# atx/padne

Measured on AMD Instinct MI355X. Metric: CG solves/s, higher is better.
Workload: dtype f64; 1 GPU; C4 8-layer N=10M: 8-layer jittered triangular Laplacian, 9999392 nodes, via-ring stitched, 1 A source/sink, amg-PCG to rtol 1e-12; n_unknowns=9999391, nnz_per_rank=69955225, rows_per_rank=9999391, parallelism=layer-partitioned x1

## Files before the change

### padne_amd/_hip.py

```python
from __future__ import annotations

import ctypes as C
import weakref
import os
import sys
from dataclasses import dataclass

import numpy as np

_HERE = os.path.dirname(os.path.abspath(__file__))
LIB_PATH = os.path.join(_HERE, "libpadne_hip.so")

OK = 0
E_INVALID, E_HIP, E_NOMEM, E_NONMANIFOLD, E_NOTCONVERGED, E_COMM, E_BREAKDOWN, E_TOOLARGE, E_NOCOARSEN = \
    -1, -2, -3, -4, -5, -6, -7, -8, -9


class HipUnavailableError(RuntimeError):
    """libpadne_hip.so cannot be loaded or no MI355X is visible."""


class HipError(RuntimeError):
    def __init__(self, code: int, message: str):
        super().__init__(f"libpadne_hip error {code}: {message}")
# ... 109 lines not shown
                                       _PF64, _PF64, _PF64]),
    "padne_sampler_stats": (C.c_int, [_P, C.c_int32, _PI64, _PF64]),
    "padne_spmv_algorithmic_bytes": (_I64, [_P]),
    "padne_spmv_time": (C.c_int, [_P, _P, _P, _P, C.c_int, C.c_int, _PF64]),
}

TEST_SIGNATURES = {
    "padne_team_create": (C.c_int, [C.c_int, C.POINTER(_P)]),
    "padne_team_destroy": (C.c_int, [_P]),
    "padne_team_abort": (C.c_int, [_P]),
    "padne_ctx_join_team": (C.c_int, [_P, _P, C.c_int]),
    "padne_csr_split_tiles": (C.c_int, [_P, C.c_int, _PI64, _PI64]),
    "padne_ctx_lockstep_groups": (C.c_int, [_P, _PI64]),
    "padne_asm_second_path_count": (C.c_int, [_PI64]),
    "padne_ctx_halo_exchange_time": (C.c_int, [_P, C.c_int32, C.POINTER(C.c_double)]),
    "padne_ctx_reload_options": (C.c_int, [_P]),
}

PROBE_SIGNATURES = {
    "padne_test_product": (C.c_int, [_P, _P, C.c_int32, _I64, C.c_int32, C.c_int32, C.c_int32, C.c_int32, _P, _P, _P, _P, _P,
                                     _P, _P, _P, _P, C.c_double, _P, _PF64, _I64, _PI32]),
}

_lib = None


def load_library(path: str | None = None) -> C.CDLL:
    global _lib
    if _lib is not None and path is None:
        return _lib
    p = path or LIB_PATH
    if not os.path.exists(p):
        raise HipUnavailableError(
            f"{p} not found: build it with `python -m padne_amd.build` (hipcc --offload-arch=gfx950). "
            "padne_amd has no CPU fallback.")
    if "torch" in sys.modules:
        pass
    try:
        lib = C.CDLL(p, mode=C.RTLD_GLOBAL)
    except OSError as exc:
        raise HipUnavailableError(f"cannot load {p}: {exc}") from exc
    for name, (res, args) in list(SIGNATURES.items()) + list(TEST_SIGNATURES.items()) + list(PROBE_SIGNATURES.items()):
        fn = getattr(lib, name)
        fn.restype = res
        fn.argtypes = args
    if lib.padne_abi_version() != 1:
        raise HipUnavailableError("libpadne_hip.so ABI version mismatch; rebuild it")
    if path is None:
        _lib = lib
    return lib


def _check(rc: int) -> None:
    if rc == OK:
        return
    msg = (load_library().padne_last_error() or b"").decode("utf-8", "replace")
    if rc == E_NONMANIFOLD:
        raise ValueError(msg or "Non-manifold mesh")
    if rc == E_INVALID:
        raise ValueError(msg)
    if rc == E_NOMEM:
        raise MemoryError(msg)
    if rc == E_TOOLARGE:
        raise OverflowError(msg)
    if rc == E_NOTCONVERGED:
# ... 811 lines not shown
        _check(self.ctx._lib.padne_csr_shape(h, C.byref(nr), C.byref(nc), C.byref(nnz)))
        indptr = np.empty(nr.value + 1, dtype=np.int32)
        indices = np.empty(nnz.value, dtype=np.int32)
        data = np.empty(nnz.value, dtype=np.float64)
        _check(self.ctx._lib.padne_csr_to_host(self.ctx._h, h, _ptr(indptr, _PI32), _ptr(indices, _PI32), _ptr(data, _PF64)))
        return sp.csr_matrix((data, indices, indptr), shape=(nr.value, nc.value))

    def amg_shapes(self):
        out = []
        for level in range(32):
            entry = {}
            for which, code in (("A", 0), ("P", 1), ("R", 2)):
                h = _P()
                if self.ctx._lib.padne_amg_level(self.ctx._h, self._h, level, code, C.byref(h)) != OK:
                    continue
                nr, nc, nnz = C.c_int64(), C.c_int64(), C.c_int64()
                _check(self.ctx._lib.padne_csr_shape(h, C.byref(nr), C.byref(nc), C.byref(nnz)))
                entry[which] = (nr.value, nc.value, nnz.value)
            if "A" not in entry:
                break
            out.append(entry)
        return out

    def split_tiles(self, level: int = -1):
        a, b = C.c_int64(), C.c_int64()
        _check(self.ctx._lib.padne_csr_split_tiles(self._h, int(level), C.byref(a), C.byref(b)))
        return a.value, b.value

    def amg_apply(self, r) -> np.ndarray:
        r = _f64(r)
        if r.shape[0] != self.shape[0]:
            raise ValueError("dimension mismatch")
        z = np.empty_like(r)
        _check(self.ctx._lib.padne_amg_apply(self.ctx._h, self._h, _ptr(r, _PF64), _ptr(z, _PF64)))
        return z

    @staticmethod
    def _opts(rtol, atol, max_iter, check_every, guess, time_spmv=False, precond="jacobi", rebuild=False) -> SolveOpts:
        pc = {"jacobi": 0, "amg": 1, 0: 0, 1: 1}[precond]
        return SolveOpts(float(rtol), float(atol), int(max_iter), pc, int(check_every),
                         (1 if guess else 0) | (2 if time_spmv else 0) | (4 if rebuild else 0))

    def solve_spd(self, b, *, rtol=1e-12, atol=0.0, max_iter=200000, check_every=0, x0=None,
                  raise_on_fail=True, precond="amg", rebuild=False) -> SolveResult:
        b = _f64(b)
        n = self.shape[0] if self.ctx.halo_n_owned is None else self.ctx.halo_n_owned
# ... 27 lines not shown
```

### padne_amd/build.py

```python
from __future__ import annotations

import os
import shutil
import subprocess
import sys

HERE = os.path.dirname(os.path.abspath(__file__))
CSRC = os.path.join(HERE, "csrc")
LIB = os.path.join(HERE, "libpadne_hip.so")
SOURCES = ["capi.hip", "spmv.hip", "spmm.hip", "pcg.hip", "assemble.hip", "comm.hip", "amg.hip", "generate.hip", "kkt.hip", "sample.hip", "error.hip", "refine.hip"]
HEADERS = ["common.hpp", "face.hpp", os.path.join("..", "..", "include", "padne_hip.h"),
           os.path.join("..", "..", "include", "padne_hip_test.h"), os.path.join("..", "..", "include", "padne_hip_probe.h")]
ARCH = "gfx950"
FLAGS = ["-O3", "-std=c++17", "-fPIC", f"--offload-arch={ARCH}", "-ffp-contract=off",
         "-fno-fast-math", "-Wall", "-Wno-unused-function", "-Wno-unused-value", "-Wno-unused-result"]


def hipcc() -> str:
    exe = shutil.which("hipcc") or "/opt/rocm/bin/hipcc"
    if not os.path.exists(exe):
        raise RuntimeError("hipcc not found: libpadne_hip.so cannot be built")
    return exe


def needs_build() -> bool:
    if not os.path.exists(LIB):
        return True
    t = os.path.getmtime(LIB)
    deps = [os.path.join(CSRC, s) for s in SOURCES + HEADERS] + [os.path.abspath(__file__)]
    return any(os.path.getmtime(d) > t for d in deps)


def build(force: bool = False, verbose: bool = True) -> str:
    if not force and not needs_build():
        return LIB
# ... 26 lines not shown
```

### padne_amd/csrc/amg.hip

```cpp
#include "common.hpp"

#include <functional>
#include <type_traits>
#include <memory>

#include <algorithm>
#include <chrono>
#include <math.h>
#include <stdlib.h>
#include <string.h>

namespace padne {

struct AmgLevel {
    const padne_csr *A = nullptr;
    padne_csr *A_owned = nullptr;
    padne_csr *P = nullptr;
    padne_csr *R = nullptr;
    padne_csr *W = nullptr;
    double lambda = 2.0;
    double jac = 0.0;
    long long n = 0;
    double *b = nullptr, *xa = nullptr, *xb = nullptr, *tmp = nullptr;
    float *b8 = nullptr, *xa8 = nullptr, *xb8 = nullptr, *tmp8 = nullptr;
    HaloPlan halo;
    int32_t *export_owned = nullptr;
    std::vector<int> export_host;
    padne_csr *P_halo = nullptr;
    float *e_ext = nullptr;
};

struct Amg {
    padne_ctx *ctx = nullptr;
    std::vector<AmgLevel> levels;
    double *coarse_inv = nullptr;
    int n_coarse = 0;
    bool f32 = false;
    float *coarse_inv32 = nullptr;
    bool dist = false;
    padne_csr *tail = nullptr;
    int n_pad = 0;
    long long tail_n = 0, tail_off = 0;
    int *seg_off = nullptr;
    double *coarse_gather = nullptr;
// ... 58 lines not shown
__device__ __forceinline__ unsigned int prio32_of(int i) {
    unsigned int h = (unsigned int)i & 0x7fffffffu;
    h = (h * 0x5bd1e995u) & 0x7fffffffu;
    h ^= h >> 15;
    h = (h * 0x2c1b3c6du) & 0x7fffffffu;
    h ^= h >> 13;
    h = (h * 0x297a2d39u) & 0x7fffffffu;
    h ^= h >> 16;
    return h + 1u;
}

__device__ __forceinline__ bool strong(double a, double di, double dj, double theta2) {
    return a * a * di * dj >= theta2;
}

__device__ __forceinline__ int xw_position(const int4 d, const int run, const int c) {
    int pos = 0;
    if (c >= d.z && c < d.z + run) pos = 2 * run + (c - d.z);
    if (c >= d.y && c < d.y + run) pos = run + (c - d.y);
    if (c >= d.x && c < d.x + run) pos = c - d.x;
    return pos;
}

__global__ __launch_bounds__(256) void strength_mark(int n, int n_wtiles, const int *__restrict__ rowptr,
                                                     const int *__restrict__ cols, const double *__restrict__ vals,
                                                     const double *__restrict__ dinv, double theta2,
                                                     int *__restrict__ scol, double *__restrict__ bound_partial,
                                                     const int4 *__restrict__ xw_desc = nullptr,
                                                     const unsigned char *__restrict__ xw_lidx = nullptr,
                                                     const int xw_run = 0, unsigned char *__restrict__ spos = nullptr,
                                                     float *__restrict__ vals32 = nullptr) {
    constexpr int CH = 512;
    __shared__ unsigned char rid_all[4 * CH];
    __shared__ double pv_all[4 * CH];
    __shared__ double red[4], red2[4];
    const int lane = threadIdx.x & 63, w = threadIdx.x >> 6;
    unsigned char *rid = rid_all + w * CH;
    double *pv = pv_all + w * CH;
    const XcdSweep sw = xcd_sweep(n_wtiles, 4, w);
    double my_max = 0.0, my_plain = 0.0;
    for (long long wt = sw.t0; wt < sw.t1; wt += sw.stride) {
        const int row0 = (int)wt * 64;
        const int row1 = min(row0 + 64, n);
        const int r = row0 + lane;
        int rs = 0, re = 0;
        double di = 0.0;
        if (r < row1) {
            rs = rowptr[r];
            re = rowptr[r + 1];
            di = dinv[r];
        }
        const int k0 = __shfl(rs, 0, 64);
        const int k1 = __shfl(re, row1 - row0 - 1, 64);
        double dF = r < row1 ? 1.0 / di : 1.0, off_strong = 0.0, off_all = 0.0, abs_all = 0.0;
        int4 dsc = make_int4(0, 0, 0, 0);
        if (spos != nullptr) dsc = xw_desc[wt];
        const bool windowed = spos != nullptr && dsc.w != 0;
        const int self_pos = windowed ? xw_position(dsc, xw_run, r) : 0;
        for (int base = k0; base < k1; base += CH) {
            const int lo = max(rs, base), hi = min(re, base + CH);
            for (int k = lo; k < hi; ++k) rid[k - base] = (unsigned char)lane;
            asm volatile("s_waitcnt lgkmcnt(0)" ::: "memory");
            __builtin_amdgcn_wave_barrier();
#pragma unroll
            for (int q = 0; q < CH / 64; ++q) {
                const int e = base + lane + 64 * q;
                const int rl = e < k1 ? rid[e - base] : 0;
                const double dr = __shfl(di, rl, 64);
                const int sp = __shfl(self_pos, rl, 64);
                if (e < k1) {
                    const int i = row0 + rl;
                    const int c = cols[e];
                    const double v = vals[e];
                    if (vals32 != nullptr) vals32[e] = (float)v;
                    const bool st = c != i && strong(v, dr, dinv[c], theta2);
                    scol[e] = st ? c : i;
                    if (windowed) spos[e] = st ? xw_lidx[e] : (unsigned char)sp;
                    if (bound_partial != nullptr) {
                        rid[e - base] = (unsigned char)(rl | (c == i ? 0x40 : 0) | (st ? 0x80 : 0));
                        pv[e - base] = v;
// ... 420 lines not shown
            for (int u = 0; u < 8; ++u) aj[u] = (k0 + u < k1 && j[u] != i) ? agg_in[j[u]] : -1;
#pragma unroll
            for (int u = 0; u < 8; ++u) {
                const double w = fabs(v[u]);
                if (aj[u] >= 0 && w > best) {
                    best = w;
                    a = aj[u];
                }
            }
        }
        for (int k = k0 + 8; k < k1; ++k) {
            const int j = scol[k];
            if (j == i) continue;
            const int aj = agg_in[j];
            if (aj < 0) continue;
            const double w = fabs(vals[k]);
            if (w > best) {
                best = w;
                a = aj;
            }
        }
    }
    agg_out[i] = a;
}

__global__ void flag_unaggregated(int n, const int *__restrict__ agg, int *__restrict__ flag) {
    const int i = blockIdx.x * blockDim.x + threadIdx.x;
    if (i < n) flag[i] = agg[i] < 0 ? 1 : 0;
}

__global__ void agg_singletons(int n, const int *__restrict__ scan, const long long *__restrict__ base_dev, int *__restrict__ agg) {
    const int i = blockIdx.x * blockDim.x + threadIdx.x;
    if (i < n && agg[i] < 0) agg[i] = (int)*base_dev + scan[i];
}

__global__ __launch_bounds__(256) void gershgorin_kernel(int n, const int *__restrict__ rowptr,
                                                         const double *__restrict__ vals,
                                                         const double *__restrict__ dinv,
                                                         double *__restrict__ partial_max) {
    __shared__ double red[256];
    double m = 0.0;
    for (int i = blockIdx.x * 256 + threadIdx.x; i < n; i += gridDim.x * 256) {
        double s = 0.0;
        for (int k = rowptr[i]; k < rowptr[i + 1]; ++k) s += fabs(vals[k]);
        s *= fabs(dinv[i]);
        m = s > m ? s : m;
// ... 1419 lines not shown
        out2[0] = red[0][0];
        out2[1] = red[1][0];
    }
}

static int gershgorin(padne_ctx *ctx, const padne_csr *A, double *lambda, bool filtered = false) {
    const int g = (int)std::min<long long>((A->n_rows + 255) / 256, 1024);
    double *part = ctx->partials + 6 * kMaxPartials;
    if (filtered)
        hipLaunchKernelGGL(gershgorin_filtered_kernel, dim3(g > 0 ? g : 1), dim3(256), 0, ctx->stream, (int)A->n_rows,
                           A->rowptr, A->cols, A->vals, A->dinv, kTheta * kTheta, part);
    else
        hipLaunchKernelGGL(gershgorin_kernel, dim3(g > 0 ? g : 1), dim3(256), 0, ctx->stream, (int)A->n_rows, A->rowptr,
                           A->vals, A->dinv, part);
    hipLaunchKernelGGL(fold_max2_kernel, dim3(1), dim3(256), 0, ctx->stream, (const double *)part, (const double *)nullptr,
                       g > 0 ? g : 1, part + kMaxPartials - 2);
    PADNE_HIP_CHECK(hipGetLastError());
    double h[2] = {0.0, 0.0};
    PADNE_TRY(read_back(ctx, part + kMaxPartials - 2, sizeof(h), h));
    double m = h[0];
    if (!(m > 0.0) || !(m < 1e6)) m = 2.0;
    *lambda = m;
    return PADNE_OK;
}

static int aggregate(padne_ctx *ctx, Scratch &sc, const padne_csr *A, int **agg_out, int *n_agg, double *lambda_f = nullptr,
                     double *lambda_plain = nullptr, unsigned char **spos_out = nullptr, int **scol_out = nullptr,
                     float *vals32_out = nullptr) {
    hipStream_t s = ctx->stream;
    const int n = (int)A->n_rows;
    const double theta2 = kTheta * kTheta;
    signed char *state = nullptr;
    unsigned int *w0 = nullptr, *w1 = nullptr, *w2 = nullptr;
    int *flag = nullptr, *scan = nullptr, *agg0 = nullptr, *agg1 = nullptr, *counter = nullptr;
    PADNE_TRY(sc.alloc(&state, (size_t)n));
    PADNE_TRY(sc.alloc(&w0, (size_t)n));
    PADNE_TRY(sc.alloc(&w1, (size_t)n));
    PADNE_TRY(sc.alloc(&w2, (size_t)n));
    PADNE_TRY(sc.alloc(&flag, (size_t)n + 1));
    PADNE_TRY(sc.alloc(&scan, (size_t)n + 1));
    PADNE_TRY(sc.alloc(&agg0, (size_t)n));
    PADNE_TRY(sc.alloc(&agg1, (size_t)n));
    constexpr int kMaxRounds = 256;
    PADNE_TRY(sc.alloc(&counter, (size_t)2 * kMaxRounds + 4));
    const dim3 g(nblk(n)), b(256);
    const int *srow = A->rowptr;
    int *scol = nullptr;
    PADNE_TRY(sc.alloc(&scol, (size_t)(A->nnz > 0 ? A->nnz : 1)));
    const int n_wt = (n + 63) / 64;
    int gm_x = std::min(2048, (n_wt + 3) / 4 > 0 ? (n_wt + 3) / 4 : 1);
    if (gm_x >= kNumXcd) gm_x -= gm_x % kNumXcd;
    const dim3 gm((unsigned)gm_x);
    double *bound_part = lambda_f != nullptr ? ctx->partials + 6 * kMaxPartials : nullptr;
    double *bound2 = nullptr;
    if (lambda_f != nullptr) PADNE_TRY(sc.alloc(&bound2, 2));
    const bool xw = A->xw_state == 1 && A->xw_run <= 85;
    unsigned char *spos = nullptr;
    if (xw) {
        PADNE_TRY(sc.alloc(&spos, (size_t)A->nnz + kPadNnz));
    }
    static_assert(kPadNnz >= 2 * kMaxRounds + 4, "one grid for everything the start clears");
    hipLaunchKernelGGL(mis_init_words, dim3(nblk(std::max(n, kPadNnz))), b, 0, s, n, w0, state, counter, 2 * kMaxRounds + 4,
                       spos != nullptr ? spos + A->nnz : (unsigned char *)nullptr, kPadNnz);
    hipLaunchKernelGGL(strength_mark, gm, b, 0, s, n, n_wt, A->rowptr, A->cols, A->vals, A->dinv, theta2, scol, bound_part,
                       xw ? A->xw_desc : (const int4 *)nullptr, xw ? (const unsigned char *)A->xw_lidx : (const unsigned char *)nullptr,
                       xw ? A->xw_run : 0, spos, vals32_out);
    PADNE_HIP_CHECK(hipGetLastError());
    const bool long_rows = !xw && n <= 65536 && A->nnz >= 24LL * n;
    auto launch_round = [&](int *open_counter) {
        if (xw) {
            hipLaunchKernelGGL((nbr_max_xw<unsigned int, false>), gm, b, 0, s, n, n_wt, srow, scol, spos, A->xw_desc, A->xw_run,
                               (const unsigned int *)w0, w1, (unsigned int *)nullptr, (signed char *)nullptr, (int *)nullptr);
            hipLaunchKernelGGL((nbr_max_xw<unsigned int, true>), gm, b, 0, s, n, n_wt, srow, scol, spos, A->xw_desc, A->xw_run,
                               (const unsigned int *)w1, (unsigned int *)nullptr, w0, state, open_counter);
        } else if (long_rows) {
            hipLaunchKernelGGL(nbr_max_wpr<unsigned int>, dim3((unsigned)((n + 3) / 4)), b, 0, s, n, srow, (const int *)scol,
                               (const unsigned int *)w0, w1);
            hipLaunchKernelGGL(nbr_max_wpr<unsigned int>, dim3((unsigned)((n + 3) / 4)), b, 0, s, n, srow, (const int *)scol,
                               (const unsigned int *)w1, w2);
            hipLaunchKernelGGL(mis_decide, dim3(std::min<unsigned>(g.x, 1024u)), b, 0, s, n, w0, w2, state, open_counter);
        } else {
            hipLaunchKernelGGL(nbr_max<unsigned int>, gm, b, 0, s, n, n_wt, srow, scol, w0, w1);
            hipLaunchKernelGGL(nbr_max<unsigned int>, gm, b, 0, s, n, n_wt, srow, scol, w1, w2);
            hipLaunchKernelGGL(mis_decide, dim3(std::min<unsigned>(g.x, 1024u)), b, 0, s, n, w0, w2, state, open_counter);
        }
    };
    if (lambda_f != nullptr)
        hipLaunchKernelGGL(fold_max2_kernel, dim3(1), dim3(256), 0, s, (const double *)bound_part,
                           (const double *)(bound_part + kMaxPartials), (int)gm.x, bound2);
    double h_bound2[2] = {0.0, 0.0};
    bool bound_pending = lambda_f != nullptr;
    auto count_back = [&](const int *dev_count, int *host_count) -> int {
        if (!bound_pending) return read_back(ctx, dev_count, sizeof(int), host_count);
        bound_pending = false;
        return read_back2(ctx, dev_count, sizeof(int), host_count, bound2, sizeof(h_bound2), h_bound2);
    };
    int open_count = n;
    int round = 0;
    const bool compact_ok = A->nnz <= 16LL * n;
    const int full_batch = n > 200000 ? 1 : 4;
    while (round < kMaxRounds && open_count > 0 && (!compact_ok || round < 2 || open_count > n / 8)) {
        const int reps = (round == 0 && compact_ok && full_batch < 2) ? 2 : full_batch;
        for (int rep = 0; rep < reps && round < kMaxRounds; ++rep, ++round) {
            launch_round(counter + round);
        }
        PADNE_HIP_CHECK(hipGetLastError());
        PADNE_TRY(count_back(counter + round - 1, &open_count));
    }
    if (open_count > 0) {
        int *list_a = (int *)w1, *list_b = (int *)w2;
        unsigned int *m2 = nullptr;
        PADNE_TRY(sc.alloc(&m2, (size_t)open_count));
// ... 18 lines not shown
                hipLaunchKernelGGL(mis_decide_list, gl, b, 0, s, counters + cur, list_a, m2, w0, state, list_b, counters + cur + 1);
                std::swap(list_a, list_b);
                ++cur;
            }
            PADNE_HIP_CHECK(hipGetLastError());
            PADNE_TRY(count_back(counters + cur, &cnt));
        }
        open_count = cnt;
    }
    PADNE_REQUIRE(open_count == 0, "independent-set rounds did not terminate");
    if (lambda_f != nullptr) {
        if (bound_pending) PADNE_TRY(read_back(ctx, bound2, sizeof(h_bound2), h_bound2));
        double m = h_bound2[0], mp = h_bound2[1];
        if (!(m > 0.0) || !(m < 1e6)) m = 2.0;
        if (!(mp > 0.0) || !(mp < 1e6)) mp = 2.0;
        *lambda_f = m;
        if (lambda_plain != nullptr) *lambda_plain = mp;
    }
    hipLaunchKernelGGL(flag_state, g, b, 0, s, n, state, flag, 1);
    ScanTicket t_roots, t_single;
    long long h_roots[2] = {0, 0}, h_single[2] = {0, 0};
    PADNE_TRY(scan_i32_begin(ctx, flag, scan, n, &t_roots, true));
    hipLaunchKernelGGL(agg_from_roots, g, b, 0, s, n, state, scan, agg0);
    hipLaunchKernelGGL(agg_join, g, b, 0, s, n, srow, scol, A->vals, agg0, agg1);
    hipLaunchKernelGGL(agg_join, g, b, 0, s, n, srow, scol, A->vals, agg1, agg0);
    hipLaunchKernelGGL(flag_unaggregated, g, b, 0, s, n, agg0, flag);
    int rc_scan = scan_i32_begin(ctx, flag, scan, n, &t_single, true);
    if (rc_scan == PADNE_OK && t_roots.bs != nullptr)
        hipLaunchKernelGGL(agg_singletons, g, b, 0, s, n, scan, (const long long *)(t_roots.bs + t_roots.nb), agg0);
    const int rc_roots = scan_i32_end(ctx, &t_roots, h_roots);
    if (rc_scan == PADNE_OK) rc_scan = scan_i32_end(ctx, &t_single, h_single);
    PADNE_TRY(rc_roots);
    PADNE_TRY(rc_scan);
    PADNE_HIP_CHECK(hipGetLastError());
    const long long n_roots = h_roots[0], n_single = h_single[0];
    PADNE_REQUIRE(n_roots >= 0 && n_single >= 0 && n_roots + n_single < 2147483647LL, "aggregate count out of range");
    *agg_out = agg0;
    *n_agg = (int)(n_roots + n_single);
    if (spos_out != nullptr) *spos_out = spos;
    if (scol_out != nullptr) *scol_out = scol;
    return PADNE_OK;
}

template <int CAP>
__global__ __launch_bounds__(128) void prolong_rows_lds(int n, const int *__restrict__ rowptr, const int *__restrict__ cols,
                                                        const double *__restrict__ vals, const double *__restrict__ dinv,
                                                        double theta2, double omega, const int *__restrict__ agg,
                                                        const int *__restrict__ slot_ptr, long long *__restrict__ key,
// ... 565 lines not shown
        keep_slots->valid = true;
        sc.disown(first);
        sc.disown(key);
        sc.disown(val);
        if (C != nullptr) *C = nullptr;
        return PADNE_OK;
    }
    auto trampoline = [](void *f) -> int { return (*static_cast<const std::function<int()> *>(f))(); };
    return csr_from_slots(ctx, n, Y->n_cols, row_begin != nullptr ? row_begin : slot_ptr, key, val, row_len, C,
                          while_multiplying != nullptr ? +trampoline : nullptr, const_cast<std::function<int()> *>(while_multiplying));
}

__global__ void slot_row_lengths(int n, const int *__restrict__ begin, const int *__restrict__ end, int *__restrict__ len) {
    const int i = blockIdx.x * blockDim.x + threadIdx.x;
    if (i < n) len[i] = end[i] - begin[i];
}

__global__ __launch_bounds__(256) void w_from_slots_kernel(int n, const int *__restrict__ ap_begin,
                                                           const long long *__restrict__ ap_key,
                                                           const double *__restrict__ ap_val, const int *__restrict__ pr,
                                                           const int *__restrict__ pc, const double *__restrict__ pv,
                                                           const double *__restrict__ dinv, const double c,
                                                           const int *__restrict__ wr, int *__restrict__ wc,
                                                           float *__restrict__ wv) {
    __shared__ int rp_all[4][65];
    __shared__ int sp_all[4][65];
    const int lane = threadIdx.x & 63, w = threadIdx.x >> 6;
    int *rp = rp_all[w], *sp = sp_all[w];
    const long long n_wt = ((long long)n + 63) / 64;
    for (long long wt = (long long)blockIdx.x * 4 + w; wt < n_wt; wt += (long long)gridDim.x * 4) {
        const long long r0 = wt * 64;
        const int nr = (int)((n - r0) < 64 ? (n - r0) : 64);
        if (lane <= nr) rp[lane] = wr[r0 + lane];
        if (lane < nr) sp[lane] = ap_begin[r0 + lane];
        if (lane == 0 && nr == 64) rp[64] = wr[r0 + 64];
        asm volatile("s_waitcnt lgkmcnt(0)" ::: "memory");
        __builtin_amdgcn_wave_barrier();
        const int d0 = rp[0], d1 = rp[nr];
        for (int k = d0 + lane; k < d1; k += 64) {
            int lo = 0, hi = nr;
            while (hi - lo > 1) {
                const int mid = (lo + hi) >> 1;
                if (rp[mid] <= k) lo = mid; else hi = mid;
            }
            const int i = (int)r0 + lo;
            const int src = sp[lo] + (k - rp[lo]);
            const int col = (int)(ap_key[src] >> 32);
            double v = -c * dinv[i] * ap_val[src];
            const I2u be = *reinterpret_cast<const I2u *>(pr + i);
            if (be.y - be.x <= 4) {
                const I4u c4 = *reinterpret_cast<const I4u *>(pc + be.x);
                const D2u p0 = *reinterpret_cast<const D2u *>(pv + be.x), p1 = *reinterpret_cast<const D2u *>(pv + be.x + 2);
                const int ln = be.y - be.x;
                if (ln > 0 && c4.x == col) v = p0.x + v;
                if (ln > 1 && c4.y == col) v = p0.y + v;
// ... 19 lines not shown
                            double c, padne_csr **W_out, int grid_cap = 0, bool with_plan = true) {
    hipStream_t s = ctx->stream;
    const int n = (int)A->n_rows;
    Scratch sc(ctx);
    int *len = nullptr;
    PADNE_TRY(sc.alloc(&len, (size_t)n + 1));
    struct CsrDrop { void operator()(padne_csr *m) const { if (m) padne_csr_destroy(m); } };
    std::unique_ptr<padne_csr, CsrDrop> w_owner(new padne_csr());
    padne_csr *W = w_owner.get();
    W->n_rows = n;
    W->n_cols = P->n_cols;
    W->nnz = n_slots;
    W->device = ctx->device;
    W->owner = ctx;
    W->hierarchy_operator = true;
    W->xw_state = -1;
    W->rowptr = (int32_t *)pool_alloc(ctx, sizeof(int32_t) * ((size_t)n + 1));
    W->cols = (int32_t *)pool_alloc(ctx, sizeof(int32_t) * ((size_t)n_slots + kPadNnz));
    W->vals32 = (float *)pool_alloc(ctx, sizeof(float) * ((size_t)n_slots + kPadNnz));
    if (!W->rowptr || !W->cols || !W->vals32) return PADNE_E_NOMEM;
    hipLaunchKernelGGL(slot_row_lengths, dim3(nblk(n)), dim3(256), 0, s, n, ap.begin, ap.end, len);
    PADNE_HIP_CHECK(hipGetLastError());
    PADNE_TRY(exclusive_scan_i32_async(ctx, len, W->rowptr, n));
    unsigned gw = nblk(((long long)n + 63) / 64, 4);
    if (grid_cap > 0 && gw > (unsigned)grid_cap) gw = (unsigned)grid_cap;
    hipLaunchKernelGGL(w_from_slots_kernel, dim3(gw), dim3(256), 0, s, n, ap.begin, ap.key, ap.val,
                       P->rowptr, P->cols, P->vals, A->dinv, c, (const int *)W->rowptr, W->cols, W->vals32);
    PADNE_HIP_CHECK(hipGetLastError());
    W->xw_state = 0;
    if (with_plan) PADNE_TRY(csr_build_xw_plan_wide(ctx, W, grid_cap));
    if (W->xw_state != 1) W->xw_state = -1;
    *W_out = w_owner.release();
    return PADNE_OK;
}

static int dense_inverse(padne_ctx *ctx, const padne_csr *A, double **inv_out) {
    hipStream_t s = ctx->stream;
    const int n = (int)A->n_rows;
    Scratch sc(ctx);
    double *W = nullptr, *W2 = nullptr, *inv = nullptr;
    PADNE_TRY(sc.alloc(&W, (size_t)n * n));
    PADNE_TRY(sc.alloc(&W2, (size_t)n * n));
    inv = (double *)pool_alloc(ctx, sizeof(double) * (size_t)(n > 0 ? n : 1) * (size_t)(n > 0 ? n : 1));
    if (inv == nullptr) return PADNE_E_NOMEM;
    if (n > 0) {
        hipLaunchKernelGGL(dense_from_csr, dim3(n), dim3(256), 0, s, n, A->rowptr, A->cols, A->vals, W);
        const dim3 ge(nblk(n), (unsigned)((n + kGjStrip - 1) / kGjStrip));
        double *src = W, *dst = W2;
        const bool mfma = !ctx->opt.gj_vector && n > kGjM;
        if (mfma) {
// ... 210 lines not shown
            if (want_f32) PADNE_TRY(csr_build_f32(aux, const_cast<padne_csr *>(A)));
            if (want_f32 && L.P != nullptr && !w_expected) PADNE_TRY(csr_build_f32(aux, L.P));
            if (want_f32 && L.R != nullptr) PADNE_TRY(csr_build_f32(aux, L.R));
            return PADNE_OK;
        };
        if (coarsest && (rc = queue_level_extras()) != PADNE_OK) { amg->levels.push_back(L); break; }
        if (coarsest) {
            amg->levels.push_back(L);
            break;
        }
        Scratch sc(ctx);
        int *agg = nullptr, n_agg = 0;
        PhaseTimer pt(ctx, amg_verbose());
        double lambda_f = 2.0;
        unsigned char *spos = nullptr;
        int *scol = nullptr;
        float *v32 = nullptr;
        if (want_f32 && A->vals32 == nullptr && A->nnz > 0) {
            padne_csr *Am = const_cast<padne_csr *>(A);
            v32 = (float *)pool_alloc(Am->owner ? Am->owner : ctx, sizeof(float) * ((size_t)A->nnz + kPadNnz));
            if (v32 == nullptr) { rc = PADNE_E_NOMEM; amg->levels.push_back(L); break; }
            Am->vals32 = v32;
        }
        if ((rc = aggregate(ctx, sc, A, &agg, &n_agg, &lambda_f, &L.lambda, &spos, &scol, v32)) != PADNE_OK) { amg->levels.push_back(L); break; }
        pt.lap("aggregate");
        if (n_agg == 0 || (double)n_agg > 0.8 * (double)A->n_rows) {
            rc = queue_level_extras();
            amg->levels.push_back(L);
            break;
        }
        if (L.lambda < lambda_f) lambda_f = L.lambda;
        const double omega = kOmegaNum / lambda_f;
        if (amg_verbose())
            fprintf(stderr, "[amg] level %d: n=%lld nnz=%lld lambda=%.3f (P: %.3f) -> %d aggregates\n", lvl,
                    (long long)A->n_rows, (long long)A->nnz, L.lambda, lambda_f, n_agg);
        padne_csr *AP = nullptr, *Ac = nullptr;
        if ((rc = build_prolongator(ctx, A, agg, n_agg, omega, &L.P, spos, scol)) != PADNE_OK) { amg->levels.push_back(L); break; }
        pt.lap("prolongator");
        if (amg_verbose()) fprintf(stderr, "[amg]   P: %lld x %lld nnz=%lld\n", (long long)L.P->n_rows, (long long)L.P->n_cols, (long long)L.P->nnz);
        if (two && (rc = stream_order(ctx, aux)) != PADNE_OK) { amg->levels.push_back(L); break; }
        const std::function<int()> queue_transpose = [&]() -> int { return transpose(aux, L.P, &L.R); };
        SlotRows ap_rows;
        if ((rc = spgemm(ctx, A, L.P, &AP, nullptr, &ap_rows, &queue_transpose)) != PADNE_OK) { amg->levels.push_back(L); break; }
        if (L.R == nullptr && (rc = transpose(aux, L.P, &L.R)) != PADNE_OK) { amg->levels.push_back(L); break; }
        pt.lap("A*P (P^T queued beside it)");
        const bool with_w = lvl == 0 && want_f32 && ap_rows.valid && ctx->opt.amg_w >= 1;
// ... 987 lines not shown
    if (!amg || level < 0 || level >= (int)amg->levels.size()) return nullptr;
    const AmgLevel &L = amg->levels[(size_t)level];
    return which == 0 ? L.A : (which == 1 ? L.P : L.R);
}

int csr_matmul(padne_ctx *ctx, const padne_csr *X, const padne_csr *Y, padne_csr **C) { return spgemm(ctx, X, Y, C); }
const padne_csr *amg_level_matrix(const padne_csr *A0, int level, int which);
int csr_transpose(padne_ctx *ctx, const padne_csr *M, padne_csr **T) { return transpose(ctx, M, T); }

void amg_info(const padne_csr *A0, int *levels, double *complexity, double *setup_seconds, long long *coarse_n) {
    const Amg *amg = (const Amg *)A0->amg;
    if (!amg) return;
    if (levels) {
        *levels = (int)amg->levels.size();
        if (amg->tail && amg->tail->amg) *levels += (int)((const Amg *)amg->tail->amg)->levels.size() - 1;
    }
    if (complexity) *complexity = amg->operator_complexity;
    if (setup_seconds) *setup_seconds = amg->setup_seconds;
    if (coarse_n) *coarse_n = amg->n_coarse;
}

}

extern "C" int padne_csr_split_tiles(const padne_csr *m, int level, int64_t *interior, int64_t *boundary) {
    PADNE_REQUIRE(m && interior && boundary, "null argument");
    const padne_csr *a = level < 0 ? m : padne::amg_level_matrix(m, level, 0);
    *interior = *boundary = 0;
    if (a != nullptr && a->split_state == 1) {
        *interior = a->split_n_int;
        *boundary = a->split_n_bnd;
    }
    return PADNE_OK;
}
```

### padne_amd/csrc/assemble.hip

```cpp
#include "common.hpp"
#include "face.hpp"

#include <atomic>

#include <cmath>

#include <algorithm>

#include <string.h>

namespace padne {

constexpr int kScanItems = 16;
constexpr int kScanChunk = 256 * kScanItems;

__device__ __forceinline__ int block_exclusive_scan_256(int v, int *lds , int *total) {
    const int lane = threadIdx.x & 63, w = threadIdx.x >> 6;
    int inc = v;
#pragma unroll
    for (int off = 1; off < 64; off <<= 1) {
        const int t = __shfl_up(inc, off, 64);
        if (lane >= off) inc += t;
    }
    if (lane == 63) lds[w] = inc;
// ... 3469 lines not shown
    double *d_xy = nullptr, *d_q = nullptr, *d_pd = nullptr;
    long long *d_pi = nullptr, *d_out = nullptr;
    int *d_pc = nullptr, *d_outc = nullptr;
    PADNE_TRY(sc.alloc(&d_pc, (size_t)n_chunks * n_query));
    PADNE_TRY(sc.alloc(&d_outc, (size_t)n_query));
    PADNE_TRY(sc.alloc(&d_xy, (size_t)2 * n_points));
    PADNE_TRY(sc.alloc(&d_q, (size_t)2 * n_query));
    PADNE_TRY(sc.alloc(&d_pd, (size_t)n_chunks * n_query));
    PADNE_TRY(sc.alloc(&d_pi, (size_t)n_chunks * n_query));
    PADNE_TRY(sc.alloc(&d_out, (size_t)n_query));
    PADNE_HIP_CHECK(hipMemcpyAsync(d_xy, xy_host, sizeof(double) * 2 * (size_t)n_points, hipMemcpyHostToDevice, s));
    PADNE_HIP_CHECK(hipMemcpyAsync(d_q, query_host, sizeof(double) * 2 * (size_t)n_query, hipMemcpyHostToDevice, s));
    hipLaunchKernelGGL(nn_chunk_kernel, dim3(n_chunks), dim3(256), 0, s, (long long)n_points, d_xy, (int)n_query, d_q, d_pd,
                       d_pi, d_pc);
    hipLaunchKernelGGL(nn_reduce_kernel, dim3(nblk(n_query)), dim3(256), 0, s, n_chunks, (int)n_query, d_pd, d_pi, d_pc, d_out,
                       d_outc);
    PADNE_HIP_CHECK(hipGetLastError());
    PADNE_HIP_CHECK(hipMemcpyAsync(index_out_host, d_out, sizeof(long long) * (size_t)n_query, hipMemcpyDeviceToHost, s));
    if (tie_count_out_host != nullptr)
        PADNE_HIP_CHECK(hipMemcpyAsync(tie_count_out_host, d_outc, sizeof(int) * (size_t)n_query, hipMemcpyDeviceToHost, s));
    PADNE_HIP_CHECK(hipStreamSynchronize(s));
    return PADNE_OK;
}
```

### padne_amd/csrc/capi.hip

```cpp
#include "common.hpp"

#include <algorithm>

#include <math.h>
#include <stdarg.h>
#include <string.h>
#include <chrono>

namespace padne {

std::atomic<long long> g_launch_count{0};

void options_from_env(padne_options *o) {
    *o = padne_options();
    auto on = [](const char *name) { const char *e = getenv(name); return e != nullptr && e[0] != '\0' && !(e[0] == '0' && e[1] == '\0'); };
    auto has = [](const char *list, const char *word) {
        const size_t n = strlen(word);
        for (const char *p = list; p != nullptr && *p != '\0';) {
            const char *q = strchr(p, ',');
            const size_t len = q != nullptr ? (size_t)(q - p) : strlen(p);
            if (len >= n && strncmp(p, word, n) == 0 && (len == n || p[n] == ':')) return p;
            p = q != nullptr ? q + 1 : nullptr;
        }
        return (const char *)nullptr;
    };
    o->amg_f64 = on("PADNE_AMG_F64");
    if (const char *e = getenv("PADNE_AMG_W")) o->amg_w = strcmp(e, "none") == 0 ? 0 : (strcmp(e, "fine") == 0 ? 1 : 2);
    o->amg_exchange_all = on("PADNE_AMG_EXCHANGE_ALL");
    o->pcg_p64 = on("PADNE_PCG_P64");
    o->pcg_no_xhist = on("PADNE_PCG_NO_XHIST");
    o->gj_vector = on("PADNE_GJ_VECTOR");
    o->no_batch = on("PADNE_NO_BATCH");
    o->no_mailbox = on("PADNE_NO_MAILBOX");
    o->no_p2p = on("PADNE_NO_P2P");
    o->no_split = on("PADNE_NO_SPLIT");
    o->no_xwindow = on("PADNE_NO_XWINDOW");
    o->setup_one_stream = on("PADNE_SETUP_ONE_STREAM");
    if (const char *e = getenv("PADNE_CG_SINGLE_REDUCTION")) o->cg_single_reduction = atoi(e) != 0 ? 1 : 0;
    if (const char *e = getenv("PADNE_LOCKSTEP_NARROW")) o->lockstep_narrow = atoi(e);
    if (const char *e = getenv("PADNE_AMG_COARSE_N")) o->amg_coarse_n = std::min(4096, std::max(16, atoi(e)));
    if (const char *e = getenv("PADNE_AMG_GATHER_N")) o->amg_gather_n = atoll(e);
    if (const char *e = getenv("PADNE_P2P_TIMEOUT_MS")) {
        const long v = atol(e);
        if (v > 0 && v <= 600000) o->p2p_timeout_ms = (unsigned)v;
    }
    if (const char *f = getenv("PADNE_FORCE")) {
        o->force_asm_hash = has(f, "asm_hash") != nullptr;
        o->force_asm_two_pass = has(f, "asm_two_pass") != nullptr;
        o->force_relabel_slots = has(f, "relabel_slots") != nullptr;
        o->force_transpose_cursors = has(f, "transpose_cursors") != nullptr;
// ... 582 lines not shown
```

### padne_amd/csrc/common.hpp

```cpp
#pragma once

#include <hip/hip_runtime.h>
#include <stdint.h>
#include <stdio.h>
#include <map>
#include <string>
#include <unordered_map>
#include <vector>

#include "../../include/padne_hip.h"
#include "../../include/padne_hip_test.h"
#include "../../include/padne_hip_probe.h"

#include <atomic>

namespace padne {

extern std::atomic<long long> g_launch_count;

void set_error(const char *fmt, ...);

#define PADNE_HIP_CHECK(expr)                                                              \
    do {                                                                                   \
        hipError_t _e = (expr);                                                            \
        if (_e != hipSuccess) {                                                            \
            ::padne::set_error("%s failed: %s (%s:%d)", #expr, hipGetErrorString(_e),      \
                               __FILE__, __LINE__);                                        \
            return PADNE_E_HIP;                                                            \
        }                                                                                  \
    } while (0)

#define PADNE_REQUIRE(cond, msg)                                                           \
    do {                                                                                   \
        if (!(cond)) {                                                                     \
            ::padne::set_error("invalid argument: %s (%s)", msg, #cond);                   \
// ... 42 lines not shown
    int device = 0;
    padne_ctx *owner = nullptr;
    void *amg = nullptr;
    float *vals32 = nullptr, *dinv32 = nullptr;
    int4 *xw_desc = nullptr;
    unsigned short *xw_lidx = nullptr;
    int xw_state = 0;
    int xw_run = 0;
    int xw_nruns = 3;
    int *split_tiles = nullptr;
    int split_n_int = 0, split_n_bnd = 0;
    int split_state = 0;
    bool hierarchy_operator = false;
    bool cols_unsorted = false;
    padne_csr *prec_block = nullptr;
    double *mesh_xy = nullptr, *mesh_sigma = nullptr;
    int32_t *mesh_tri = nullptr;
    long long *mesh_voff = nullptr, *mesh_toff = nullptr;
    int64_t mesh_n_vert = 0, mesh_n_tri = 0, mesh_n_mesh = 0;
};

struct padne_options {
    bool amg_f64 = false;
    int amg_w = 2;
    bool amg_exchange_all = false;
    bool pcg_p64 = false;
    bool pcg_no_xhist = false;
    bool gj_vector = false;
    bool no_batch = false;
    bool no_mailbox = false;
    bool no_p2p = false;
    bool no_split = false;
    bool no_xwindow = false;
    bool setup_one_stream = false;
    int cg_single_reduction = -1;
    int lockstep_narrow = -1;
    int amg_coarse_n = 2048;
    long long amg_gather_n = 0;
    unsigned p2p_timeout_ms = 20000;
    bool force_asm_hash = false, force_asm_two_pass = false, force_relabel_slots = false, force_transpose_cursors = false;
    bool force_relabel_lanes = false;
    bool force_xhist_small = false;
    long long force_spgemm_split = 0;
    bool verbose_amg = false, verbose_xw = false, verbose_pool = false;
};
namespace padne { void options_from_env(padne_options *o); }
// ... 205 lines not shown
```

Before: 31.86 solves/s.

## Adapt rows-per-wave in AMG setup kernels by level size and density

```diff
diff --git a/include/padne_hip_setup_probe.h b/include/padne_hip_setup_probe.h
--- /dev/null
+++ b/include/padne_hip_setup_probe.h
@@ -0,0 +1,17 @@
+#ifndef PADNE_HIP_SETUP_PROBE_H
+#define PADNE_HIP_SETUP_PROBE_H
+
+#include "padne_hip.h"
+
+#ifdef __cplusplus
+extern "C" {
+#endif
+
+int padne_amg_rows_per_wave(const padne_csr *m, int level, int32_t *rows);
+int padne_test_exclusive_scan(padne_ctx *ctx, const int32_t *in_host, int64_t n, int32_t *out_host, int64_t *total);
+
+#ifdef __cplusplus
+}
+#endif
+
+#endif
diff --git a/padne_amd/_hip.py b/padne_amd/_hip.py
--- a/padne_amd/_hip.py
+++ b/padne_amd/_hip.py
@@ -155,6 +155,11 @@
                                      _P, _P, _P, _P, C.c_double, _P, _PF64, _I64, _PI32]),
 }
 
+SETUP_PROBE_SIGNATURES = {
+    "padne_amg_rows_per_wave": (C.c_int, [_P, C.c_int, _PI32]),
+    "padne_test_exclusive_scan": (C.c_int, [_P, _PI32, _I64, _PI32, _PI64]),
+}
+
 _lib = None
 
 
@@ -173,7 +178,8 @@
         lib = C.CDLL(p, mode=C.RTLD_GLOBAL)
     except OSError as exc:
         raise HipUnavailableError(f"cannot load {p}: {exc}") from exc
-    for name, (res, args) in list(SIGNATURES.items()) + list(TEST_SIGNATURES.items()) + list(PROBE_SIGNATURES.items()):
+    for name, (res, args) in list(SIGNATURES.items()) + list(TEST_SIGNATURES.items()) + list(PROBE_SIGNATURES.items()) + \
+            list(SETUP_PROBE_SIGNATURES.items()):
         fn = getattr(lib, name)
         fn.restype = res
         fn.argtypes = args
@@ -1031,6 +1037,14 @@
             out.append(entry)
         return out
 
+    def amg_rows_per_wave(self):
+        out = []
+        for level in range(len(self.amg_shapes())):
+            r = C.c_int32()
+            _check(self.ctx._lib.padne_amg_rows_per_wave(self._h, level, C.byref(r)))
+            out.append(int(r.value))
+        return out
+
     def split_tiles(self, level: int = -1):
         a, b = C.c_int64(), C.c_int64()
         _check(self.ctx._lib.padne_csr_split_tiles(self._h, int(level), C.byref(a), C.byref(b)))
diff --git a/padne_amd/build.py b/padne_amd/build.py
--- a/padne_amd/build.py
+++ b/padne_amd/build.py
@@ -10,7 +10,8 @@
 LIB = os.path.join(HERE, "libpadne_hip.so")
 SOURCES = ["capi.hip", "spmv.hip", "spmm.hip", "pcg.hip", "assemble.hip", "comm.hip", "amg.hip", "generate.hip", "kkt.hip", "sample.hip", "error.hip", "refine.hip"]
 HEADERS = ["common.hpp", "face.hpp", os.path.join("..", "..", "include", "padne_hip.h"),
-           os.path.join("..", "..", "include", "padne_hip_test.h"), os.path.join("..", "..", "include", "padne_hip_probe.h")]
+           os.path.join("..", "..", "include", "padne_hip_test.h"), os.path.join("..", "..", "include", "padne_hip_probe.h"),
+           os.path.join("..", "..", "include", "padne_hip_setup_probe.h")]
 ARCH = "gfx950"
 FLAGS = ["-O3", "-std=c++17", "-fPIC", f"--offload-arch={ARCH}", "-ffp-contract=off",
          "-fno-fast-math", "-Wall", "-Wno-unused-function", "-Wno-unused-value", "-Wno-unused-result"]
diff --git a/padne_amd/csrc/amg.hip b/padne_amd/csrc/amg.hip
--- a/padne_amd/csrc/amg.hip
+++ b/padne_amd/csrc/amg.hip
@@ -20,6 +20,7 @@
     padne_csr *W = nullptr;
     double lambda = 2.0;
     double jac = 0.0;
+    int rows_per_wave = 64;
     long long n = 0;
     double *b = nullptr, *xa = nullptr, *xb = nullptr, *tmp = nullptr;
     float *b8 = nullptr, *xa8 = nullptr, *xb8 = nullptr, *tmp8 = nullptr;
@@ -124,6 +125,7 @@
     return pos;
 }
 
+template <int TR>
 __global__ __launch_bounds__(256) void strength_mark(int n, int n_wtiles, const int *__restrict__ rowptr,
                                                      const int *__restrict__ cols, const double *__restrict__ vals,
                                                      const double *__restrict__ dinv, double theta2,
@@ -142,8 +144,8 @@
     const XcdSweep sw = xcd_sweep(n_wtiles, 4, w);
     double my_max = 0.0, my_plain = 0.0;
     for (long long wt = sw.t0; wt < sw.t1; wt += sw.stride) {
-        const int row0 = (int)wt * 64;
-        const int row1 = min(row0 + 64, n);
+        const int row0 = (int)wt * TR;
+        const int row1 = min(row0 + TR, n);
         const int r = row0 + lane;
         int rs = 0, re = 0;
         double di = 0.0;
@@ -156,8 +158,8 @@
         const int k1 = __shfl(re, row1 - row0 - 1, 64);
         double dF = r < row1 ? 1.0 / di : 1.0, off_strong = 0.0, off_all = 0.0, abs_all = 0.0;
         int4 dsc = make_int4(0, 0, 0, 0);
-        if (spos != nullptr) dsc = xw_desc[wt];
-        const bool windowed = spos != nullptr && dsc.w != 0;
+        if (TR == 64 && spos != nullptr) dsc = xw_desc[wt];
+        const bool windowed = TR == 64 && spos != nullptr && dsc.w != 0;
         const int self_pos = windowed ? xw_position(dsc, xw_run, r) : 0;
         for (int base = k0; base < k1; base += CH) {
             const int lo = max(rs, base), hi = min(re, base + CH);
@@ -624,6 +626,46 @@
         }
     }
     agg_out[i] = a;
+}
+
+template <int LG>
+__global__ __launch_bounds__(256) void agg_join_lanes(int n, const int *__restrict__ srow, const int *__restrict__ scol,
+                                                      const double *__restrict__ vals, const int *__restrict__ agg_in,
+                                                      int *__restrict__ agg_out) {
+    const long long g = ((long long)blockIdx.x * 256 + threadIdx.x) / LG;
+    const int sub = threadIdx.x % LG;
+    const bool live = g < n;
+    const int i = live ? (int)g : 0;
+    const int a = live ? agg_in[i] : 0;
+    const bool open = live && a < 0;
+    double best = -1.0;
+    int kbest = 0x7fffffff, abest = a;
+    if (open) {
+        const int k0 = srow[i], k1 = srow[i + 1];
+        for (int k = k0 + sub; k < k1; k += LG) {
+            const int j = scol[k];
+            if (j == i) continue;
+            const int aj = agg_in[j];
+            if (aj < 0) continue;
+            const double w = fabs(vals[k]);
+            if (w > best) {
+                best = w;
+                abest = aj;
+                kbest = k;
+            }
+        }
+    }
+#pragma unroll
+    for (int off = LG / 2; off > 0; off >>= 1) {
+        const double ow = __shfl_xor(best, off, 64);
+        const int ok = __shfl_xor(kbest, off, 64), oa = __shfl_xor(abest, off, 64);
+        if (ow > best || (ow == best && ok < kbest)) {
+            best = ow;
+            kbest = ok;
+            abest = oa;
+        }
+    }
+    if (live && sub == 0) agg_out[i] = abest;
 }
 
 __global__ void flag_unaggregated(int n, const int *__restrict__ agg, int *__restrict__ flag) {
@@ -2089,6 +2131,14 @@
     if (!(m > 0.0) || !(m < 1e6)) m = 2.0;
     *lambda = m;
     return PADNE_OK;
+}
+
+static int setup_rows_per_wave(const padne_ctx *ctx, long long n, long long nnz, bool windowed) {
+    const int form = ctx->opt.amg_row_form;
+    if (windowed || n <= 0 || form == 1) return 64;
+    const int lanes = (nnz >= 48 * n || n <= 32768) ? 4 : 16;
+    if (form == 2) return lanes;
+    return (n > 262144 || nnz < 12 * n) ? 64 : lanes;
 }
 
 static int aggregate(padne_ctx *ctx, Scratch &sc, const padne_csr *A, int **agg_out, int *n_agg, double *lambda_f = nullptr,
@@ -2129,9 +2179,21 @@
     static_assert(kPadNnz >= 2 * kMaxRounds + 4, "one grid for everything the start clears");
     hipLaunchKernelGGL(mis_init_words, dim3(nblk(std::max(n, kPadNnz))), b, 0, s, n, w0, state, counter, 2 * kMaxRounds + 4,
                        spos != nullptr ? spos + A->nnz : (unsigned char *)nullptr, kPadNnz);
-    hipLaunchKernelGGL(strength_mark, gm, b, 0, s, n, n_wt, A->rowptr, A->cols, A->vals, A->dinv, theta2, scol, bound_part,
-                       xw ? A->xw_desc : (const int4 *)nullptr, xw ? (const unsigned char *)A->xw_lidx : (const unsigned char *)nullptr,
-                       xw ? A->xw_run : 0, spos, vals32_out);
+    const int tr = setup_rows_per_wave(ctx, n, A->nnz, xw);
+    const int n_st = (n + tr - 1) / tr;
+    int gs_x = std::min(2048, (n_st + 3) / 4 > 0 ? (n_st + 3) / 4 : 1);
+    if (gs_x >= kNumXcd) gs_x -= gs_x % kNumXcd;
+    const dim3 gs((unsigned)gs_x);
+    if (tr == 64)
+        hipLaunchKernelGGL(strength_mark<64>, gs, b, 0, s, n, n_st, A->rowptr, A->cols, A->vals, A->dinv, theta2, scol, bound_part,
+                           xw ? A->xw_desc : (const int4 *)nullptr, xw ? (const unsigned char *)A->xw_lidx : (const unsigned char *)nullptr,
+                           xw ? A->xw_run : 0, spos, vals32_out);
+    else if (tr == 16)
+        hipLaunchKernelGGL(strength_mark<16>, gs, b, 0, s, n, n_st, A->rowptr, A->cols, A->vals, A->dinv, theta2, scol, bound_part,
+                           (const int4 *)nullptr, (const unsigned char *)nullptr, 0, (unsigned char *)nullptr, vals32_out);
+    else
+        hipLaunchKernelGGL(strength_mark<4>, gs, b, 0, s, n, n_st, A->rowptr, A->cols, A->vals, A->dinv, theta2, scol, bound_part,
+                           (const int4 *)nullptr, (const unsigned char *)nullptr, 0, (unsigned char *)nullptr, vals32_out);
     PADNE_HIP_CHECK(hipGetLastError());
     const bool long_rows = !xw && n <= 65536 && A->nnz >= 24LL * n;
     auto launch_round = [&](int *open_counter) {
@@ -2154,7 +2216,7 @@
     };
     if (lambda_f != nullptr)
         hipLaunchKernelGGL(fold_max2_kernel, dim3(1), dim3(256), 0, s, (const double *)bound_part,
-                           (const double *)(bound_part + kMaxPartials), (int)gm.x, bound2);
+                           (const double *)(bound_part + kMaxPartials), (int)gs.x, bound2);
     double h_bound2[2] = {0.0, 0.0};
     bool bound_pending = lambda_f != nullptr;
     auto count_back = [&](const int *dev_count, int *host_count) -> int {
@@ -2219,8 +2281,13 @@
     long long h_roots[2] = {0, 0}, h_single[2] = {0, 0};
     PADNE_TRY(scan_i32_begin(ctx, flag, scan, n, &t_roots, true));
     hipLaunchKernelGGL(agg_from_roots, g, b, 0, s, n, state, scan, agg0);
-    hipLaunchKernelGGL(agg_join, g, b, 0, s, n, srow, scol, A->vals, agg0, agg1);
-    hipLaunchKernelGGL(agg_join, g, b, 0, s, n, srow, scol, A->vals, agg1, agg0);
+    auto launch_join = [&](const int *from, int *to) {
+        if (tr == 64) hipLaunchKernelGGL(agg_join, g, b, 0, s, n, srow, scol, A->vals, from, to);
+        else if (tr == 16) hipLaunchKernelGGL(agg_join_lanes<4>, dim3(nblk((long long)n * 4)), b, 0, s, n, srow, (const int *)scol, A->vals, from, to);
+        else hipLaunchKernelGGL(agg_join_lanes<16>, dim3(nblk((long long)n * 16)), b, 0, s, n, srow, (const int *)scol, A->vals, from, to);
+    };
+    launch_join(agg0, agg1);
+    launch_join(agg1, agg0);
     hipLaunchKernelGGL(flag_unaggregated, g, b, 0, s, n, agg0, flag);
     int rc_scan = scan_i32_begin(ctx, flag, scan, n, &t_single, true);
     if (rc_scan == PADNE_OK && t_roots.bs != nullptr)
@@ -2832,15 +2899,15 @@
                                                            const int *__restrict__ pc, const double *__restrict__ pv,
                                                            const double *__restrict__ dinv, const double c,
                                                            const int *__restrict__ wr, int *__restrict__ wc,
-                                                           float *__restrict__ wv) {
+                                                           float *__restrict__ wv, const int rpw) {
     __shared__ int rp_all[4][65];
     __shared__ int sp_all[4][65];
     const int lane = threadIdx.x & 63, w = threadIdx.x >> 6;
     int *rp = rp_all[w], *sp = sp_all[w];
-    const long long n_wt = ((long long)n + 63) / 64;
+    const long long n_wt = ((long long)n + rpw - 1) / rpw;
     for (long long wt = (long long)blockIdx.x * 4 + w; wt < n_wt; wt += (long long)gridDim.x * 4) {
-        const long long r0 = wt * 64;
-        const int nr = (int)((n - r0) < 64 ? (n - r0) : 64);
+        const long long r0 = wt * rpw;
+        const int nr = (int)((n - r0) < rpw ? (n - r0) : rpw);
         if (lane <= nr) rp[lane] = wr[r0 + lane];
         if (lane < nr) sp[lane] = ap_begin[r0 + lane];
         if (lane == 0 && nr == 64) rp[64] = wr[r0 + 64];
@@ -2906,10 +2973,11 @@
     hipLaunchKernelGGL(slot_row_lengths, dim3(nblk(n)), dim3(256), 0, s, n, ap.begin, ap.end, len);
     PADNE_HIP_CHECK(hipGetLastError());
     PADNE_TRY(exclusive_scan_i32_async(ctx, len, W->rowptr, n));
-    unsigned gw = nblk(((long long)n + 63) / 64, 4);
+    const int rpw = setup_rows_per_wave(ctx, n, n_slots, false);
+    unsigned gw = nblk(((long long)n + rpw - 1) / rpw, 4);
     if (grid_cap > 0 && gw > (unsigned)grid_cap) gw = (unsigned)grid_cap;
     hipLaunchKernelGGL(w_from_slots_kernel, dim3(gw), dim3(256), 0, s, n, ap.begin, ap.key, ap.val,
-                       P->rowptr, P->cols, P->vals, A->dinv, c, (const int *)W->rowptr, W->cols, W->vals32);
+                       P->rowptr, P->cols, P->vals, A->dinv, c, (const int *)W->rowptr, W->cols, W->vals32, rpw);
     PADNE_HIP_CHECK(hipGetLastError());
     W->xw_state = 0;
     if (with_plan) PADNE_TRY(csr_build_xw_plan_wide(ctx, W, grid_cap));
@@ -3166,6 +3234,7 @@
             if (v32 == nullptr) { rc = PADNE_E_NOMEM; amg->levels.push_back(L); break; }
             Am->vals32 = v32;
         }
+        L.rows_per_wave = setup_rows_per_wave(ctx, A->n_rows, A->nnz, A->xw_state == 1 && A->xw_run <= 85);
         if ((rc = aggregate(ctx, sc, A, &agg, &n_agg, &lambda_f, &L.lambda, &spos, &scol, v32)) != PADNE_OK) { amg->levels.push_back(L); break; }
         pt.lap("aggregate");
         if (n_agg == 0 || (double)n_agg > 0.8 * (double)A->n_rows) {
@@ -4199,6 +4268,14 @@
 
 }
 
+extern "C" int padne_amg_rows_per_wave(const padne_csr *m, int level, int32_t *rows) {
+    PADNE_REQUIRE(m && rows, "null argument");
+    const padne::Amg *amg = (const padne::Amg *)m->amg;
+    PADNE_REQUIRE(amg != nullptr && level >= 0 && level < (int)amg->levels.size(), "no such multigrid level");
+    *rows = amg->levels[(size_t)level].rows_per_wave;
+    return PADNE_OK;
+}
+
 extern "C" int padne_csr_split_tiles(const padne_csr *m, int level, int64_t *interior, int64_t *boundary) {
     PADNE_REQUIRE(m && interior && boundary, "null argument");
     const padne_csr *a = level < 0 ? m : padne::amg_level_matrix(m, level, 0);
diff --git a/padne_amd/csrc/assemble.hip b/padne_amd/csrc/assemble.hip
--- a/padne_amd/csrc/assemble.hip
+++ b/padne_amd/csrc/assemble.hip
@@ -3515,3 +3515,19 @@
     PADNE_HIP_CHECK(hipStreamSynchronize(s));
     return PADNE_OK;
 }
+
+extern "C" int padne_test_exclusive_scan(padne_ctx *ctx, const int32_t *in_host, int64_t n, int32_t *out_host, int64_t *total) {
+    using namespace padne;
+    PADNE_REQUIRE(ctx && out_host && total && n >= 0 && (in_host || n == 0), "null argument");
+    PADNE_HIP_CHECK(hipSetDevice(ctx->device));
+    hipStream_t s = ctx->stream;
+    Scratch sc(ctx);
+    int *d_in = nullptr, *d_out = nullptr;
+    PADNE_TRY(sc.alloc(&d_in, (size_t)n));
+    PADNE_TRY(sc.alloc(&d_out, (size_t)n + 1));
+    if (n > 0) PADNE_HIP_CHECK(hipMemcpyAsync(d_in, in_host, sizeof(int32_t) * (size_t)n, hipMemcpyHostToDevice, s));
+    PADNE_TRY(exclusive_scan_i32(ctx, d_in, d_out, n, total));
+    PADNE_HIP_CHECK(hipMemcpyAsync(out_host, d_out, sizeof(int32_t) * ((size_t)n + 1), hipMemcpyDeviceToHost, s));
+    PADNE_HIP_CHECK(hipStreamSynchronize(s));
+    return PADNE_OK;
+}
diff --git a/padne_amd/csrc/capi.hip b/padne_amd/csrc/capi.hip
--- a/padne_amd/csrc/capi.hip
+++ b/padne_amd/csrc/capi.hip
@@ -26,6 +26,7 @@
     };
     o->amg_f64 = on("PADNE_AMG_F64");
     if (const char *e = getenv("PADNE_AMG_W")) o->amg_w = strcmp(e, "none") == 0 ? 0 : (strcmp(e, "fine") == 0 ? 1 : 2);
+    if (const char *e = getenv("PADNE_AMG_ROW_FORM")) o->amg_row_form = strcmp(e, "thread") == 0 ? 1 : (strcmp(e, "wave") == 0 ? 2 : 0);
     o->amg_exchange_all = on("PADNE_AMG_EXCHANGE_ALL");
     o->pcg_p64 = on("PADNE_PCG_P64");
     o->pcg_no_xhist = on("PADNE_PCG_NO_XHIST");
diff --git a/padne_amd/csrc/common.hpp b/padne_amd/csrc/common.hpp
--- a/padne_amd/csrc/common.hpp
+++ b/padne_amd/csrc/common.hpp
@@ -11,6 +11,7 @@
 #include "../../include/padne_hip.h"
 #include "../../include/padne_hip_test.h"
 #include "../../include/padne_hip_probe.h"
+#include "../../include/padne_hip_setup_probe.h"
 
 #include <atomic>
 
@@ -99,6 +100,7 @@
 
 struct padne_options {
     bool amg_f64 = false;
+    int amg_row_form = 0;
     int amg_w = 2;
     bool amg_exchange_all = false;
     bool pcg_p64 = false;
```

Result: no change. 31.85 solves/s, median of 2 (-0.0%).
